# spcl/gms

Measured on AMD Instinct MI355X. Metric: edges-intersected/sec + achieved HBM GB/s, RMAT-26 triangle count @1/2/4/8 GPU, higher is better.
Workload: dtype int32 ids / uint64 counts

## Files before the change

### gms_amd/csrc/hip/device_graph.hip

```cpp
#include "device_graph.hpp"

#include <algorithm>
#include <mutex>
#include <array>
#include <chrono>
#include <cstdio>
#include <cstdlib>
#include <cstring>
#include <memory>
#include <new>
#include <random>

#include <rocprim/device/device_radix_sort.hpp>
#include <rocprim/device/device_scan.hpp>
#include <rocprim/device/device_segmented_radix_sort.hpp>
#include <rocprim/iterator/transform_iterator.hpp>

#include "../host/gmsx_internal.hpp"
#include "../host/tc_core_plan.hpp"
#include "kc4_mfma.hpp"

namespace gmsx {

Ctx &ctx() {
// ... 576 lines not shown
    uint32_t *c = cnt + p * kClasses;
    uint32_t run = 0;
    for (int k = 0; k < hub_end; ++k) { const uint32_t x = c[k]; c[k] = run; run += x; }
    hcnt[p] = run;
    run = 0;
    for (int k = hub_end; k < kClasses; ++k) { const uint32_t x = c[k]; c[k] = run; run += x; }
    tcnt[p] = run;
}

__global__ void k_ledge_count(int64_t first, int64_t end, const int32_t *__restrict__ order, const int64_t *__restrict__ toff, const int32_t *__restrict__ tadj,
                              const int32_t *__restrict__ tsplit, const int32_t *__restrict__ dplus, int32_t core, int64_t *__restrict__ cnt) {
    const int64_t pos = first + int64_t(blockIdx.x) * blockDim.x + threadIdx.x;
    if (pos > end) return;
    int64_t c = 0;
    if (pos < end) {
        const int32_t u = order[pos];
        const int64_t tb = toff[u];
        const int tl = int(toff[u + 1] - tb);
        if (u >= core)
            for (int i = tsplit[u]; i < tl; ++i) c += dplus[tadj[tb + i]] < kHeavy ? 1 : 0;
    }
    cnt[pos - first] = c;
}
__global__ void k_ledge_fill(int64_t first, int64_t end, const int32_t *__restrict__ order, const int64_t *__restrict__ hoff, const int64_t *__restrict__ toff,
                             const int32_t *__restrict__ tadj, const int32_t *__restrict__ tsplit, const int32_t *__restrict__ dplus,
                             int32_t core, const int64_t *__restrict__ ebeg, int nparts, int part, uint4 *__restrict__ ledge) {
    const int64_t pos = first + int64_t(blockIdx.x) * blockDim.x + threadIdx.x;
    if (pos >= end) return;
    const int32_t u = order[pos];
    if (u < core) return;
    const int64_t hb = hoff[u], tb = toff[u];
    const int tl = int(toff[u + 1] - tb);
    const unsigned long long hu = (unsigned long long)hb | ((unsigned long long)(hoff[u + 1] - hb) << 40);
    int64_t e = ebeg[pos - first];
    for (int i = tsplit[u]; i < tl; ++i) {
        const int32_t v = tadj[tb + i];
        if (dplus[v] >= kHeavy) continue;
        if (nparts <= 1 || shard_of(e, nparts) == part) {
            const unsigned long long tu = (unsigned long long)tb | ((unsigned long long)i << 40);
            const unsigned long long hv = (unsigned long long)hoff[v] | ((unsigned long long)(hoff[v + 1] - hoff[v]) << 40);
            const unsigned long long tv = (unsigned long long)toff[v] | ((unsigned long long)(toff[v + 1] - toff[v]) << 40);
            const int64_t slot = nparts <= 1 ? e : e / nparts;
            ledge[2 * slot] = make_uint4(uint32_t(hu), uint32_t(hu >> 32), uint32_t(tu), uint32_t(tu >> 32));
            ledge[2 * slot + 1] = make_uint4(uint32_t(hv), uint32_t(hv >> 32), uint32_t(tv), uint32_t(tv >> 32));
        }
        ++e;
    }
}

__device__ __forceinline__ uint32_t cut_hub_units(const uint32_t *__restrict__ spool, unsigned long long d, int below, int32_t v) {
    const uint32_t units = uint32_t(d) & 0x3fffffu, form = (uint32_t(d) >> 22) & 3u;
    if (form == kFormList) return min(units, uint32_t(below + 7) / 8u);
    if (form == kFormBitset) return min(units, uint32_t(v + 127) / 128u);
    const uint4 *row = reinterpret_cast<const uint4 *>(spool) + (d >> 24);
    uint32_t lo = 0, hi = units;
    while (lo < hi) {
        const uint32_t mid = (lo + hi) >> 1;
        if (int32_t(row[mid].x & 0xffffu) < v) lo = mid + 1; else hi = mid;
    }
    return lo;
}
__device__ __forceinline__ uint32_t cut_tail_units(const uint32_t *__restrict__ tpool, unsigned long long d, int below, int32_t v) {
    const uint32_t units = uint32_t(d) & 0x3fffffu, form = (uint32_t(d) >> 22) & 3u;
    if (form != kFormDelta) return min(units, uint32_t(below + 3) / 4u);
    const uint4 *row = reinterpret_cast<const uint4 *>(tpool) + (d >> 24);
    uint32_t lo = 0, hi = units;
    while (lo < hi) {
// ... 162 lines not shown
        *p = nullptr;
        return GMSX_ERR_DEVICE_MEM;
    }
    if (hipMalloc(reinterpret_cast<void **>(p), bytes) != hipSuccess) {
        (void)hipGetLastError();
        *p = nullptr;
        return GMSX_ERR_DEVICE_MEM;
    }
    if (g) g->device_bytes += int64_t(bytes);
    return GMSX_OK;
}

struct DevGuard {
    void *p;
    ~DevGuard() { (void)hipFree(p); }
};

static void free_tc(gmsx_graph *g) {
    auto drop = [](auto *&p) {
        (void)hipFree(p);
        p = nullptr;
    };
    drop(g->tsplit); drop(g->srow); drop(g->srow2); drop(g->ksplit); drop(g->spool); drop(g->trow); drop(g->htask.lo); drop(g->htask.hi); drop(g->ttask.lo); drop(g->ttask.hi); drop(g->hitem); drop(g->titem); drop(g->tunits);
    drop(g->ledge); drop(g->tpool); drop(g->shard_hitem); drop(g->shard_titem); drop(g->core_bits);
    g->tc_core = 0;
    g->shard_idx_part = g->shard_idx_nparts = -1;
    g->device_bytes -= g->tc_bytes;
    g->tc_bytes = 0;
    g->tc_ready = false;
    g->htask_entries = g->ttask_entries = g->hitems = g->titems = g->inline_hentries = g->inline_tentries = 0;
    g->n_ledge = g->ledge_total = 0;
    g->task_reverse = g->inline_units = g->spool_units = g->tpool_units = 0;
    g->stats_part = g->stats_nparts = -1;
}

static void free_graph(gmsx_graph *g) {
    if (!g) return;
    (void)hipFree(g->off);
    (void)hipFree(g->adj);
    (void)hipFree(g->newid);
    (void)hipFree(g->oldid);
    (void)hipFree(g->hoff);
    (void)hipFree(g->hadj);
    (void)hipFree(g->toff);
    (void)hipFree(g->tadj);
    (void)hipFree(g->bmoff);
    (void)hipFree(g->bmpool);
    (void)hipFree(g->tsplit);
    (void)hipFree(g->srow);
    (void)hipFree(g->srow2);
    (void)hipFree(g->ksplit);
    (void)hipFree(g->spool);
    (void)hipFree(g->trow);
    (void)hipFree(g->htask.lo);
    (void)hipFree(g->htask.hi);
    (void)hipFree(g->ttask.lo);
    (void)hipFree(g->ttask.hi);
    (void)hipFree(g->hitem);
    (void)hipFree(g->titem);
    (void)hipFree(g->tunits);
    (void)hipFree(g->shard_hitem);
    (void)hipFree(g->shard_titem);
    (void)hipFree(g->ledge);
    (void)hipFree(g->core_bits);
    (void)hipFree(g->tpool);
    (void)hipFree(g->dplus);
    (void)hipFree(g->order);
    (void)hipFree(g->kc_rel);
    (void)hipFree(g->kc_aoff);
    (void)hipFree(g->kc_arena);
    (void)hipFree(g->kc_rec);
    (void)hipFree(g->kc_item);
    (void)hipFree(g->kc_relt);
    (void)hipFree(g->kc_rect);
    (void)hipFree(g->kc_itemt);
    (void)hipFree(g->scratch);
    (void)hipFree(g->acc);
    delete g;
}

int exclusive_scan_i64(const int64_t *in, int64_t *out, int64_t count, hipStream_t s) {
    size_t tmp_bytes = 0;
    GMSX_HIP(rocprim::exclusive_scan(nullptr, tmp_bytes, in, out, int64_t(0), size_t(count), rocprim::plus<int64_t>(), s));
    void *tmp = nullptr;
    GMSX_HIP(hipMalloc(&tmp, tmp_bytes ? tmp_bytes : 8));
    DevGuard g_tmp{tmp};
// ... 502 lines not shown
        GMSX_HIP(hipMemcpy(&small_units, soff + n, sizeof(int64_t), hipMemcpyDeviceToHost));
        inline_t_base = big_units + small_units;
        g->tpool_units = inline_t_base + inline_t_units;
        if (g->tpool_units >= (int64_t(1) << 40)) return GMSX_ERR_DEVICE_MEM;
        if (int rc = dmalloc(&g->trow, n, g)) return rc;
        if (int rc = dmalloc(&g->tpool, (g->tpool_units + kPoolSlack) * 4, g)) return rc;
        GMSX_HIP(hipMemsetD32Async(reinterpret_cast<hipDeviceptr_t>(g->tpool), int(0xFFFFFFFEu), size_t(g->tpool_units + kPoolSlack) * 4, s));
        if (n > 0)
            hipLaunchKernelGGL(k_trow_fill, dim3(unsigned((n + 255) / 256)), dim3(256), 0, s, n, g->toff, g->tadj, uoff, soff, real, form, g->trow, g->tpool);
        GMSX_HIP(hipStreamSynchronize(s));
    }

    pt.mark("tail stream rows");
    if (n_work > 0) {
        GMSX_HIP(hipMemsetAsync(inl_h, 0, size_t(n + 1) * sizeof(unsigned long long), s));
        GMSX_HIP(hipMemsetAsync(inl_t, 0, size_t(n + 1) * sizeof(unsigned long long), s));
        hipLaunchKernelGGL(k_inline_rows<true>, dim3(grid_for_waves(n_work)), dim3(256), 0, s, int64_t(0), n_work, g->order, g->hoff, g->hadj, g->toff,
                           g->tadj, g->dplus, g->inline_limit, g->inline_first, g->tc_core, opos, g->shard_nparts, g->shard_part, inl_h, inl_t, ihoff, itoff, inline_h_base, reinterpret_cast<uint16_t *>(g->spool),
                           inline_t_base, reinterpret_cast<int32_t *>(g->tpool));
    }
    pt.mark("inline rows fill");
    {
        const int64_t nl = n_work - n_heavy;
        g->n_ledge = g->ledge_total = 0;
        if (nl > 0) {
            int64_t *ecnt = nullptr, *ebeg = nullptr;
            if (int rc = dmalloc(&ecnt, nl + 1, nullptr)) return rc;
            DevGuard g_ec{ecnt};
            if (int rc = dmalloc(&ebeg, nl + 1, nullptr)) return rc;
            DevGuard g_eb{ebeg};
            hipLaunchKernelGGL(k_ledge_count, dim3(unsigned(nl / 256 + 1)), dim3(256), 0, s, n_heavy, n_work, g->order, g->toff, g->tadj, g->tsplit, g->dplus, g->tc_core, ecnt);
            if (int rc = exclusive_scan_i64(ecnt, ebeg, nl + 1, s)) return rc;
            GMSX_HIP(hipMemcpy(&g->ledge_total, ebeg + nl, sizeof(int64_t), hipMemcpyDeviceToHost));
            const int np = g->shard_nparts > 1 ? g->shard_nparts : 1, pp = g->shard_nparts > 1 ? g->shard_part : 0;
            {
                const int64_t full = g->ledge_total / np, rem = g->ledge_total % np;
                g->n_ledge = np <= 1 ? g->ledge_total : full + (((full & 1) ? np - 1 - pp : pp) < rem ? 1 : 0);
            }
            if (int rc = dmalloc(&g->ledge, 2 * g->n_ledge + 2, g)) return rc;
            hipLaunchKernelGGL(k_ledge_fill, dim3(unsigned(nl / 256 + 1)), dim3(256), 0, s, n_heavy, n_work, g->order, g->hoff, g->toff, g->tadj, g->tsplit, g->dplus, g->tc_core, ebeg,
                               np, pp, g->ledge);
            GMSX_HIP(hipStreamSynchronize(s));
        }
    }
    pt.mark("light pivot list");
    {
        int two_sided = 1;
        if (const char *e = opt("TC_TWO_SIDED")) two_sided = std::atoi(e) != 0;
        const unsigned vb = unsigned(n / 256 + 1);
        const int64_t L = g->inline_limit;
        int64_t *lflag = nullptr, *lidx = nullptr;
        if (int rc = dmalloc(&lflag, L + 1, nullptr)) return rc;
        DevGuard g_lf{lflag};
        if (int rc = dmalloc(&lidx, L + 1, nullptr)) return rc;
        DevGuard g_li{lidx};
        hipLaunchKernelGGL(k_light_flags, dim3(unsigned(L / 256 + 1)), dim3(256), 0, s, L, g->dplus, lflag);
        if (int rc = exclusive_scan_i64(lflag, lidx, L + 1, s)) return rc;
        int64_t n_light_recv = 0;
        GMSX_HIP(hipMemcpy(&n_light_recv, lidx + L, sizeof(int64_t), hipMemcpyDeviceToHost));
        const int64_t n_recv = n_heavy + n_light_recv;
        int32_t *recv_v = nullptr;
        if (int rc = dmalloc(&recv_v, n_recv + 1, nullptr)) return rc;
        DevGuard g_rv{recv_v};
        if (std::max<int64_t>(n_heavy, L) > 0)
// ... 388 lines not shown
```

### gms_amd/csrc/hip/device_graph.hpp

```cpp
#pragma once
#include <hip/hip_runtime.h>

#include <cstdint>

#include "gmsx.h"
#include "gmsx_internal.hpp"

#if !defined(GMSX_DEV_HOOKS) &&                                                                                                               \
    (defined(GMSX_KC_NO_PROBE) || defined(GMSX_KC_NO_HITS) || defined(GMSX_KC_NO_TAIL) || defined(GMSX_KC_NO_INNER) || defined(GMSX_KC_CELLS_ONLY) ||   \
     defined(GMSX_KC_NO_ROWS) || defined(GMSX_KC_BUILD_ONLY) || defined(GMSX_KC_NO_SLAB_CALL) || defined(GMSX_KC_NO_PAIRS) || defined(GMSX_KC_SLAB_ROW_SCAN) || \
     defined(GMSX_BK_AB) || defined(GMSX_BK_NO_HIT_ATOMICS) || defined(GMSX_BK_STATS) || defined(GMSX_TC_NO_PROBE) || defined(GMSX_TC_STAGING_ONLY))
#error "A/B switches need -DGMSX_DEV_HOOKS (tools/ab_lib.sh sets it); the default build of libgmsx.so carries none of them"
#endif

struct __attribute__((aligned(64))) gmsx_tc_item {
    uint64_t bc;
    uint64_t cont;
    int32_t pivot;
    int32_t pos;
    uint32_t kind;
    uint16_t fbeg[4];
    uint32_t reserved[7];
};
static_assert(sizeof(gmsx_tc_item) == 64, "work item record = one 64-byte line");
constexpr uint32_t kTaskHubUnitsMax = (1u << 14) - 1, kTaskTailUnitsMax = (1u << 15) - 1;
struct TaskList {
    uint32_t *lo = nullptr;
    uint16_t *hi = nullptr;
    bool tail = false;
// ... 20 lines not shown
    uint16_t *hadj = nullptr;
    int64_t *toff = nullptr;
    int32_t *tadj = nullptr;
    int64_t *bmoff = nullptr;
    uint32_t *bmpool = nullptr;
    int32_t dense_limit = 0;
    int32_t bitset_limit = 0;
    unsigned long long *srow = nullptr;
    unsigned long long *srow2 = nullptr;
    int32_t *ksplit = nullptr;
    uint32_t *spool = nullptr;
    int64_t spool_units = 0;
    TaskList htask{nullptr, nullptr, false};
    TaskList ttask{nullptr, nullptr, true};
    int64_t htask_entries = 0, ttask_entries = 0;
    struct gmsx_tc_item *hitem = nullptr, *titem = nullptr;
    int64_t hitems = 0, titems = 0;
    int64_t inline_hentries = 0, inline_tentries = 0;
    mutable struct gmsx_tc_item *shard_hitem = nullptr, *shard_titem = nullptr;
    mutable int64_t shard_hitems = 0, shard_titems = 0;
    mutable int shard_idx_part = -1, shard_idx_nparts = -1;
    int32_t *tunits = nullptr;
    int64_t task_reverse = 0;
    uint4 *ledge = nullptr;
    int64_t n_ledge = 0, ledge_total = 0;
    uint32_t *core_bits = nullptr;
    int32_t tc_core = 0;
    mutable int core_bytes_k = -1, core_bytes_part = -1, core_bytes_nparts = -1;
    mutable uint64_t core_bytes = 0;
    int tc_hot_windows = 0;
    uint32_t tc_window_units = 1;
    int tc_hot_min = 0;
    int inline_first = 64;
    int32_t inline_limit = 0;
    int64_t inline_units = 0;
    unsigned long long *trow = nullptr;
    uint32_t *tpool = nullptr;
    int64_t tpool_units = 0;
    int32_t *tsplit = nullptr;
    int64_t dense_rows = 0, bmpool_words = 0;
    bool rows_sorted = false;
    int32_t *dplus = nullptr;
    int32_t *order = nullptr;
    int64_t hub_entries = 0, tail_entries = 0;
    int32_t max_dplus = 0;
    int32_t max_deg = 0;
    mutable bool kc_rev_tried = false;
    mutable uint32_t *kc_rel = nullptr;
// ... 89 lines not shown
    hipStream_t side[2] = {nullptr, nullptr};
    hipEvent_t ev_fork = nullptr, ev_join[2] = {nullptr, nullptr};
    int compute_units = 0;
};
Ctx &ctx();
int ensure_init();
int kclique_vertex_counts(const gmsx_graph *g, unsigned long long *d_counts, gmsx_stats *st);
int count_dplus_ge(const gmsx_graph *g, int32_t threshold, int64_t *out);
int exclusive_scan_i64(const int64_t *in, int64_t *out, int64_t count, hipStream_t s);
int ensure_tc(const gmsx_graph *g);
int ensure_tc_shard(const gmsx_graph *g, int part, int nparts);
int tc_shard_items(const gmsx_graph *g, int part, int nparts);
int tc_vertex_counts_device(const gmsx_graph *g, unsigned long long *d_counts, gmsx_stats *st);
int tc_full_partial(const gmsx_graph *g, int part, int nparts, uint64_t *partial, gmsx_stats *st);

__device__ __forceinline__ int uni32(int x) { return __builtin_amdgcn_readfirstlane(x); }
__device__ __forceinline__ uint32_t uni32(uint32_t x) { return uint32_t(__builtin_amdgcn_readfirstlane(int(x))); }
__device__ __forceinline__ int64_t uni64(int64_t x) {
    const uint32_t lo = uint32_t(__builtin_amdgcn_readfirstlane(int(uint32_t(uint64_t(x)))));
    const uint32_t hi = uint32_t(__builtin_amdgcn_readfirstlane(int(uint32_t(uint64_t(x) >> 32))));
    return int64_t((uint64_t(hi) << 32) | lo);
}
__device__ __forceinline__ unsigned long long uni64(unsigned long long x) { return (unsigned long long)uni64(int64_t(x)); }

#define GMSX_HIP(call)                                                    \
    do {                                                                  \
        hipError_t e_ = (call);                                           \
        if (e_ != hipSuccess) {                                           \
            (void)hipGetLastError();                                      \
            return e_ == hipErrorOutOfMemory ? GMSX_ERR_DEVICE_MEM : GMSX_ERR_KERNEL; \
        }                                                                 \
    } while (0)

}
```

### gms_amd/csrc/hip/tc.hip

```cpp
#include "device_graph.hpp"
#include "kc4_mfma.hpp"
#include "../host/tc_core_plan.hpp"

#include <algorithm>
#include <type_traits>
#include <rocprim/device/device_radix_sort.hpp>
#include <rocprim/device/device_reduce.hpp>
#include <rocprim/device/device_reduce_by_key.hpp>
#include <cstdio>
#include <cstdlib>
#include <cstring>

namespace gmsx {

static constexpr int kAccSlots = 64;
static constexpr int kAccStride = 16;

struct __attribute__((packed, aligned(4))) u4u { uint32_t x, y, z, w; };

__device__ __forceinline__ int64_t readlane64(int64_t x, int l) {
    const uint32_t lo = __builtin_amdgcn_readlane(uint32_t(uint64_t(x)), l);
    const uint32_t hi = __builtin_amdgcn_readlane(uint32_t(uint64_t(x) >> 32), l);
    return int64_t((uint64_t(hi) << 32) | lo);
}
// ... 511 lines not shown
__global__ __launch_bounds__(256) __attribute__((amdgpu_waves_per_eu(TAIL ? GMSX_TC_TAIL_MIN_WAVES : GMSX_TC_HUB_MIN_WAVES, 8))) void k_tc_items(
    const uint16_t *__restrict__ hadj, const int32_t *__restrict__ tadj, const uint32_t *__restrict__ pool, const TaskList task,
    const gmsx_tc_item *__restrict__ items, int n_items, unsigned int *__restrict__ qhead, unsigned long long *__restrict__ acc) {
    __shared__ __attribute__((aligned(16))) ItemLds L;
    const int tid = threadIdx.x;
    unsigned long long total = 0;
    item_loop<TAIL>(L, hadj, tadj, pool, task, items, n_items, qhead, total);
    block_add(total, L.red, tid & 63, tid >> 6, tid, acc);
}

template <int K>
__device__ __forceinline__ uint32_t ror_in_row(uint32_t x) {
    if constexpr (K == 0) return x;
    else return uint32_t(__builtin_amdgcn_mov_dpp(int(x), 0x120 + K, 0xf, 0xf, false));
}
__device__ __forceinline__ bool row_has(uint32_t a, uint32_t x) {
    bool m = false;
#define GMSX_ROT(K) m |= a == ror_in_row<K>(x);
    GMSX_ROT(0) GMSX_ROT(1) GMSX_ROT(2) GMSX_ROT(3) GMSX_ROT(4) GMSX_ROT(5) GMSX_ROT(6) GMSX_ROT(7)
    GMSX_ROT(8) GMSX_ROT(9) GMSX_ROT(10) GMSX_ROT(11) GMSX_ROT(12) GMSX_ROT(13) GMSX_ROT(14) GMSX_ROT(15)
#undef GMSX_ROT
    return m;
}
struct LightRows {
    uint32_t ah[4], at[4], bh[4], bt[4];
};
struct LightRec {
    uint4 r0, r1;
};
__global__ __launch_bounds__(256) void k_tc_light(const uint16_t *__restrict__ hadj, const int32_t *__restrict__ tadj, const uint4 *__restrict__ ledge, int nparts,
                                                  int part, int64_t count, unsigned long long *__restrict__ acc) {
    __shared__ unsigned long long red[4];
    const int tid = threadIdx.x, lane = tid & 63, wave = tid >> 6, sub = lane & 15;
    const int64_t ngroups = int64_t(gridDim.x) * 16, g0 = int64_t(blockIdx.x) * 16 + (tid >> 4);
    const int64_t trips = (count + ngroups - 1) / ngroups;
    auto load_rec = [&](int64_t t) -> LightRec {
        const int64_t k = g0 + t * ngroups;
        const int64_t kk = k < count ? k : 0;
        const int64_t e = nparts <= 1 ? kk : kk * nparts + ((kk & 1) ? nparts - 1 - part : part);
        LightRec r;
        r.r0 = ledge[2 * e];
        r.r1 = ledge[2 * e + 1];
        if (k >= count) {
            r.r0.y &= 0xffu;
            r.r0.w &= 0xffu;
            r.r1.y &= 0xffu;
            r.r1.w &= 0xffu;
        }
        return r;
    };
    auto wave_max = [](int x) {
        return max(max(__builtin_amdgcn_readlane(x, 0), __builtin_amdgcn_readlane(x, 16)), max(__builtin_amdgcn_readlane(x, 32), __builtin_amdgcn_readlane(x, 48)));
    };
    auto load_rows = [&](const LightRec &r) -> LightRows {
        const int64_t hu = int64_t((uint64_t(r.r0.y & 0xffu) << 32) | r.r0.x), tu = int64_t((uint64_t(r.r0.w & 0xffu) << 32) | r.r0.z);
        const int64_t hv = int64_t((uint64_t(r.r1.y & 0xffu) << 32) | r.r1.x), tv = int64_t((uint64_t(r.r1.w & 0xffu) << 32) | r.r1.z);
        const int hlu = int(r.r0.y >> 8), tlu = int(r.r0.w >> 8), hlv = int(r.r1.y >> 8), tlv = int(r.r1.w >> 8);
        const int more = wave_max((max(max(hlu, hlv), max(tlu, tlv)) + 15) >> 4);
        LightRows w;
        w.ah[0] = hadj[hlu ? hu + min(sub, hlu - 1) : 0];
        w.bh[0] = hadj[hlv ? hv + min(sub, hlv - 1) : 0];
        w.at[0] = uint32_t(tadj[tlu ? tu + min(sub, tlu - 1) : 0]);
        w.bt[0] = uint32_t(tadj[tlv ? tv + min(sub, tlv - 1) : 0]);
#pragma unroll
        for (int k = 1; k < 4; ++k) {
            w.ah[k] = w.bh[k] = w.at[k] = w.bt[k] = 0;
            if (k < more) {
                const int i = sub + 16 * k;
                w.ah[k] = hadj[hlu ? hu + min(i, hlu - 1) : 0];
                w.bh[k] = hadj[hlv ? hv + min(i, hlv - 1) : 0];
                w.at[k] = uint32_t(tadj[tlu ? tu + min(i, tlu - 1) : 0]);
                w.bt[k] = uint32_t(tadj[tlv ? tv + min(i, tlv - 1) : 0]);
            }
        }
        return w;
    };
    unsigned long long total = 0;
    if (trips > 0) {
        LightRec rec = load_rec(0);
        LightRows rows = load_rows(rec);
        LightRec rec_n = load_rec(1);
        for (int64_t t = 0; t < trips; ++t) {
            const LightRows rows_n = load_rows(rec_n);
            const LightRec rec_nn = load_rec(t + 2);
            const int hlu = int(rec.r0.y >> 8), tlu = int(rec.r0.w >> 8), hlv = int(rec.r1.y >> 8), tlv = int(rec.r1.w >> 8);
            const int nah = wave_max((hlu + 15) >> 4), nbh = wave_max((hlv + 15) >> 4), nat = wave_max((tlu + 15) >> 4), nbt = wave_max((tlv + 15) >> 4);
            uint32_t c = 0;
#pragma unroll
            for (int ka = 0; ka < 4; ++ka) {
                if (ka >= nah) break;
                const int ia = sub + 16 * ka;
                const uint32_t a = (ia < hlu && rows.ah[ka] != 0xFFFFu) ? rows.ah[ka] : 0xFFFFFFFFu;
                bool m = false;
#pragma unroll
                for (int kb = 0; kb < 4; ++kb) {
                    if (kb >= nbh) break;
                    const int ib = sub + 16 * kb;
                    const uint32_t x = (ib < hlv && rows.bh[kb] != 0xFFFFu) ? rows.bh[kb] : 0xFFFFFFFEu;
                    m |= row_has(a, x);
                }
                c += m ? 1u : 0u;
            }
#pragma unroll
            for (int ka = 0; ka < 4; ++ka) {
                if (ka >= nat) break;
                const int ia = sub + 16 * ka;
                const uint32_t a = ia < tlu ? rows.at[ka] : 0xFFFFFFFFu;
                bool m = false;
#pragma unroll
                for (int kb = 0; kb < 4; ++kb) {
                    if (kb >= nbt) break;
                    const int ib = sub + 16 * kb;
                    const uint32_t x = ib < tlv ? rows.bt[kb] : 0xFFFFFFFEu;
                    m |= row_has(a, x);
                }
                c += m ? 1u : 0u;
            }
            total += c;
            rec = rec_n;
            rows = rows_n;
            rec_n = rec_nn;
        }
    }
    block_add(total, red, lane, wave, tid, acc);
}

__global__ __launch_bounds__(1024) void k_tc_core(const uint32_t *__restrict__ bits, int WS, int K, int nb, int nblk, int part, int nparts,
                                                  unsigned long long *__restrict__ acc) {
    __shared__ unsigned long long red[16];
    auto lane_id = [] { return int(__builtin_amdgcn_mbcnt_hi(~0u, __builtin_amdgcn_mbcnt_lo(~0u, 0u))); };
    const int wave = uni32(int(threadIdx.x) >> 6);
    const int x = blockIdx.x & 7, y = blockIdx.x >> 3, Y = int(gridDim.x) >> 3;
    const int Q = 16 * Y, q = y * 16 + wave;
    const int ns = (nblk - part + nparts - 1) / nparts;
    uint32_t cnt = 0;
    for (int j = 0;; ++j) {
        const int sidx = (8 * j + ((j & 1) ? 7 - x : x)) * Q + q;
        if (sidx >= ns) break;
        const int t = sidx * nparts + part;
        int c = int((__builtin_sqrtf(8.0f * float(t) + 1.0f) - 1.0f) * 0.5f);
        while (c * (c + 1) / 2 > t) --c;
        while ((c + 1) * (c + 2) / 2 <= t) ++c;
        const int bj = nb - 1 - c, bi = bj + (t - c * (c + 1) / 2);
        int lane = lane_id();
// ... 20 lines not shown
    const int lane = threadIdx.x & 63;
    const int64_t wave0 = (int64_t(blockIdx.x) * blockDim.x + threadIdx.x) >> 6;
    const int64_t nwaves = (int64_t(gridDim.x) * blockDim.x) >> 6;
    unsigned long long units = 0, probes = 0, bytes = 0;
    for (int64_t pos = wave0; pos < end; pos += nwaves) {
        if (nparts > 1 && shard_of(pos, nparts) != part) continue;
        const int32_t u = order[pos];
        const int du = dplus[u];
        if (du >= kHeavy) {
            if (lane == 0) units += (unsigned long long)tunits[pos];
            if (u < core) {
                if (lane == 0) units += (unsigned long long)du;
                continue;
            }
            const int hl = min(int(hoff[u + 1] - hoff[u]), inline_first), tl = min(int(toff[u + 1] - toff[u]), inline_first - hl);
            int32_t v = -1;
            if (lane < hl) {
                const uint32_t x = hadj[hoff[u] + lane];
                if (x != 0xFFFFu) v = int32_t(x);
            } else if (lane - hl < tl) v = tadj[toff[u] + lane - hl];
            if (v >= 0 && lane > 0 && (v < inline_limit || dplus[v] >= kHeavy)) ++units;
            continue;
        }
        const int hl = int(hoff[u + 1] - hoff[u]);
        if (lane == 0) units += (unsigned long long)du;
        if (du < 2 || u < core) continue;
        for (int64_t j = toff[u] + lane; j < toff[u + 1]; j += 64) {
            const int32_t v = tadj[j];
            if (v < inline_limit || dplus[v] >= kHeavy) continue;
            const unsigned long long hv = (unsigned long long)(hoff[v + 1] - hoff[v]), tv = (unsigned long long)(toff[v + 1] - toff[v]);
            bytes += 32ull + 2ull * hl + 4ull * (unsigned long long)(j - toff[u]) + 2ull * hv + 4ull * tv;
            probes += hv + tv;
        }
    }
    for (int s = 32; s > 0; s >>= 1) {
        units += __shfl_down(units, s);
        probes += __shfl_down(probes, s);
        bytes += __shfl_down(bytes, s);
    }
    if (lane == 0) {
        if (units) atomicAdd(&out[0], units);
        if (probes) atomicAdd(&out[1], probes);
        if (bytes) atomicAdd(&out[2], bytes);
    }
}
__global__ __launch_bounds__(256) void k_tc_item_stats(const int64_t *__restrict__ coff, int bytes_per_id, int tail, const TaskList task,
                                                       const gmsx_tc_item *__restrict__ items, int64_t n_items, int nparts, int part,
                                                       unsigned long long *__restrict__ out) {
    const int lane = threadIdx.x & 63;
    const int64_t wave0 = (int64_t(blockIdx.x) * blockDim.x + threadIdx.x) >> 6;
    const int64_t nwaves = (int64_t(gridDim.x) * blockDim.x) >> 6;
    unsigned long long probes = 0, bytes = 0;
    auto slots = [tail](unsigned long long d) -> unsigned long long {
        const unsigned long long n = d & 0x3fffffull, f = (d >> 22) & 3ull;
// ... 1 lines not shown
    };
    for (int64_t q = wave0; q < n_items; q += nwaves) {
        const gmsx_tc_item &it = items[q];
        if (nparts > 1 && shard_of(it.pos, nparts) != part) continue;
        const int ne = int(it.bc >> 40);
        const int64_t b = int64_t(it.bc & 0xffffffffffull);
        if (lane == 0) bytes += (unsigned long long)bytes_per_id * (unsigned long long)(coff[it.pivot + 1] - coff[it.pivot]);
        for (int i = lane; i < ne; i += 64) {
            const unsigned long long d = task.get(b + i);
            bytes += 6ull + 16ull * (d & 0x3fffffull);
            probes += slots(d);
        }
    }
    for (int s = 32; s > 0; s >>= 1) {
        probes += __shfl_down(probes, s);
        bytes += __shfl_down(bytes, s);
    }
    if (lane == 0) {
        if (probes) atomicAdd(&out[1], probes);
        if (bytes) atomicAdd(&out[2], bytes);
    }
}

__global__ __launch_bounds__(256) void k_tc_breakdown(const int64_t *__restrict__ hoff, const int64_t *__restrict__ toff, const int32_t *__restrict__ tadj,
                                                      const int32_t *__restrict__ dplus, const int32_t *__restrict__ order,
                                                      const TaskList htask, const gmsx_tc_item *__restrict__ hitem, int64_t hitems,
                                                      const TaskList ttask, const gmsx_tc_item *__restrict__ titem, int64_t titems,
                                                      int32_t inline_limit, int32_t core, int64_t first_light, int64_t end_light,
                                                      unsigned long long *__restrict__ out) {
    const int lane = threadIdx.x & 63;
    const int64_t wave0 = (int64_t(blockIdx.x) * blockDim.x + threadIdx.x) >> 6;
    const int64_t nwaves = (int64_t(gridDim.x) * blockDim.x) >> 6;
    unsigned long long c[15] = {0, 0, 0, 0, 0, 0, 0, 0, 0, 0, 0, 0, 0, 0, 0};
    for (int64_t q = wave0; q < hitems + titems; q += nwaves) {
        const bool tail = q >= hitems;
        const gmsx_tc_item &it = tail ? titem[q - hitems] : hitem[q];
        const TaskList task = tail ? ttask : htask;
        const int ne = int(it.bc >> 40);
        const int64_t b0 = int64_t(it.bc & 0xffffffffffull);
        if (lane == 0) {
            c[6] += tail ? 4ull * (unsigned long long)(toff[it.pivot + 1] - toff[it.pivot]) : 2ull * (unsigned long long)(hoff[it.pivot + 1] - hoff[it.pivot]);
            c[11] += (unsigned long long)ne;
            c[13] += 1;
        }
        for (int i = lane; i < ne; i += 64) {
            const unsigned long long d = task.get(b0 + i);
            const unsigned long long db = 16ull * (d & 0x3fffffull);
            const int fd = int((d >> 22) & 3);
            if (tail) c[fd == kFormDelta ? 4 : 3] += db;
            else c[fd == kFormList ? 0 : fd == kFormBitset ? 1 : 2] += db;
            c[5] += 6;
        }
    }
    for (int64_t pos = first_light + wave0; pos < end_light; pos += nwaves) {
        const int32_t u = order[pos];
        if (u < core) continue;
        const int64_t tb0 = toff[u], te = toff[u + 1];
        const unsigned long long hl = (unsigned long long)(hoff[u + 1] - hoff[u]);
        for (int64_t j = tb0 + lane; j < te; j += 64) {
            const int32_t v = tadj[j];
            if (v < inline_limit || dplus[v] >= kHeavy) continue;
            c[8] += 2ull * (unsigned long long)(hoff[v + 1] - hoff[v]);
            c[9] += 4ull * (unsigned long long)(toff[v + 1] - toff[v]);
            c[10] += 32ull + 2ull * hl + 4ull * (unsigned long long)(j - tb0);
            c[14] += 1;
        }
    }
    for (int k = 0; k < 15; ++k) {
        unsigned long long x = c[k];
        for (int s = 32; s > 0; s >>= 1) x += __shfl_down(x, s);
        if (lane == 0 && x) atomicAdd(&out[k], x);
    }
}

__device__ __forceinline__ int hist_bin(unsigned long long units) {
    if (units <= 16) return int(units) - 1;
    int b = 16;
    for (unsigned long long lim = 32; units > lim && b < 23; lim <<= 1) ++b;
    return b;
}
__global__ __launch_bounds__(256) void k_tc_comember_keys(const TaskList htask, const gmsx_tc_item *__restrict__ hitem, int64_t hitems, int batch,
                                                         unsigned long long *__restrict__ keys, uint32_t *__restrict__ vals, unsigned long long *__restrict__ sums) {
    unsigned long long ents = 0, units = 0;
    for (int64_t i = blockIdx.x; i < hitems; i += gridDim.x) {
        const gmsx_tc_item it = hitem[i];
        const unsigned long long first = it.bc & 0xffffffffffull;
        const int n = int(it.bc >> 40);
// ... 234 lines not shown
        auto grid = [&](int64_t n, int wgs) {
            return unsigned(std::max<int64_t>(1, std::min<int64_t>((n + kGrab - 1) / kGrab, int64_t(cus) * (wgs_env > 0 ? wgs_env : wgs))));
        };
        if (n_hitems > 0) {
            hipLaunchKernelGGL(k_tc_items<false>, dim3(grid(n_hitems, GMSX_TC_HUB_MIN_WAVES)), dim3(256), 0, s, g->hadj, g->tadj, g->spool, g->htask, hitem, int(n_hitems), qhead, acc);
            ++launches;
        }
        if (n_titems > 0) {
            hipLaunchKernelGGL(k_tc_items<true>, dim3(grid(n_titems, GMSX_TC_TAIL_MIN_WAVES)), dim3(256), 0, s, g->hadj, g->tadj, g->tpool, g->ttask, titem, int(n_titems),
                               qhead + kQueueStride, acc);
            ++launches;
        }
    } else {
        if (n_hitems > 0) {
            hipLaunchKernelGGL(k_tc_block, dim3(unsigned(n_hitems)), dim3(256), 0, s, g->hoff, g->hadj, g->spool, g->htask, hitem, acc);
            ++launches;
        }
        if (n_titems > 0) {
            hipLaunchKernelGGL(k_tc_tail, dim3(unsigned(n_titems)), dim3(256), 0, side_tail ? c.side[0] : s, g->toff, g->tadj, g->tpool, g->ttask, titem, acc);
            ++launches;
        }
    }
    if (cnt_light > 0) {
        const int64_t blocks = std::min<int64_t>((cnt_light + 15) / 16, int64_t(cus) * 8);
        hipLaunchKernelGGL(k_tc_light, dim3(unsigned(blocks)), dim3(256), 0, side_light ? c.side[1] : s, g->hadj, g->tadj, g->ledge, strided ? nparts : 1,
                           strided ? part : 0, cnt_light, acc);
        ++launches;
    }
    for (int i = 0; i < 2; ++i)
        if (join.armed[i]) {
            join.armed[i] = false;
            GMSX_HIP(hipEventRecord(c.ev_join[i], c.side[i]));
            GMSX_HIP(hipStreamWaitEvent(s, c.ev_join[i], 0));
        }
    GMSX_HIP(hipEventRecord(c.ev[2], s));
    GMSX_HIP(hipGetLastError());

    const bool need_stats = st && !(g->stats_part == part && g->stats_nparts == nparts);
    if (need_stats) {
        if (g->n > 0) {
            const int64_t blocks = std::min<int64_t>((g->n + 3) / 4, cap_blocks);
            hipLaunchKernelGGL(k_tc_stats, dim3(unsigned(blocks)), dim3(256), 0, s, g->hoff, g->hadj, g->toff, g->tadj, g->dplus, g->order,
                               g->tunits, g->inline_limit, g->inline_first, g->tc_core, g->n, nparts, part, acc + kAccSlots * kAccStride);
        }
        if (g->hitems > 0)
            hipLaunchKernelGGL(k_tc_item_stats, dim3(unsigned(std::min<int64_t>((g->hitems + 3) / 4, cap_blocks))), dim3(256), 0, s, g->hoff, 2, 0, g->htask, g->hitem,
                               g->hitems, nparts, part, acc + kAccSlots * kAccStride);
        if (g->titems > 0)
// ... 33 lines not shown

using namespace gmsx;

extern "C" {

int gmsx_tc_divisor(int algo) { return algo == GMSX_TC_FULL ? 3 : 1; }

int gmsx_tc_stream_breakdown(const gmsx_graph *g, uint64_t *out21) {
    return gmsx::guard([&]() -> int {
        if (!g || !out21) return GMSX_ERR_INVALID;
        if (int rc = ensure_init()) return rc;
        if (int rc = ensure_tc(g)) return rc;
        hipStream_t s = ctx().stream;
        std::memset(out21, 0, 21 * sizeof(uint64_t));
        if (g->n == 0) return GMSX_OK;
        int64_t n_block = 0, n_work = 0;
        if (int rc = count_dplus_ge(g, kHeavy, &n_block)) return rc;
        if (int rc = count_dplus_ge(g, 2, &n_work)) return rc;
        unsigned long long *acc = nullptr;
        GMSX_HIP(hipMalloc(reinterpret_cast<void **>(&acc), 21 * 8));
        struct Guard { void *p; ~Guard() { (void)hipFree(p); } } g1{acc};
        GMSX_HIP(hipMemsetAsync(acc, 0, 21 * 8, s));
        const int cus = ctx().compute_units > 0 ? ctx().compute_units : 256;
        hipLaunchKernelGGL(k_tc_breakdown, dim3(unsigned(cus * 16)), dim3(256), 0, s, g->hoff, g->toff, g->tadj, g->dplus, g->order, g->htask,
                           g->hitem, g->hitems, g->ttask, g->titem, g->titems, g->inline_limit, g->tc_core, n_block, n_work, acc);
        GMSX_HIP(hipMemcpyAsync(out21, acc, 21 * 8, hipMemcpyDeviceToHost, s));
        GMSX_HIP(hipStreamSynchronize(s));
        GMSX_HIP(hipGetLastError());
        out21[7] = uint64_t(g->inline_units) * 16ull;
        out21[12] = uint64_t(g->inline_hentries + g->inline_tentries);
        out21[15] = core_bytes_of(g, 0, 1);
        out21[16] = uint64_t(g->tc_core);
        return GMSX_OK;
    });
}

int gmsx_tc_row_histogram(const gmsx_graph *g, uint64_t *out256) {
    return gmsx::guard([&]() -> int {
        uint64_t *out248 = out256;
        if (!g || !out248) return GMSX_ERR_INVALID;
        if (int rc = ensure_init()) return rc;
        if (int rc = ensure_tc(g)) return rc;
        hipStream_t s = ctx().stream;
        std::memset(out248, 0, 256 * sizeof(uint64_t));
        if (g->n == 0) return GMSX_OK;
        unsigned long long *acc = nullptr;
        GMSX_HIP(hipMalloc(reinterpret_cast<void **>(&acc), 256 * 8));
// ... 91 lines not shown
```

Baseline: 16.11 billion.

## Pack light-edge rows into contiguous pooled records with compact descriptors

Preprocessing now copies each light edge's four neighbor row slices (hub u, tail prefix u, hub v, tail v) into one contiguous packed record in a new pool, indexed by an 8-byte descriptor. Before, a 32-byte record pointed into the scattered hadj/tadj arrays. The light kernel now reads one descriptor plus one contiguous record instead of gathering from four scattered rows. This targets random-access gather cost and over-fetch. It also strips hub sentinels at build time, double-buffers the loop, and sizes the grid by queried occupancy. In exchange it duplicates adjacency data, which costs more memory and preprocessing time, and caps row lengths at 8 bits.

```diff
diff --git a/gms_amd/csrc/hip/device_graph.hip b/gms_amd/csrc/hip/device_graph.hip
--- a/gms_amd/csrc/hip/device_graph.hip
+++ b/gms_amd/csrc/hip/device_graph.hip
@@ -622,27 +622,55 @@
     }
     cnt[pos - first] = c;
 }
-__global__ void k_ledge_fill(int64_t first, int64_t end, const int32_t *__restrict__ order, const int64_t *__restrict__ hoff, const int64_t *__restrict__ toff,
-                             const int32_t *__restrict__ tadj, const int32_t *__restrict__ tsplit, const int32_t *__restrict__ dplus,
-                             int32_t core, const int64_t *__restrict__ ebeg, int nparts, int part, uint4 *__restrict__ ledge) {
+__global__ void k_ledge_units(int64_t first, int64_t end, const int32_t *__restrict__ order, const int64_t *__restrict__ hoff, const uint16_t *__restrict__ hadj,
+                              const int64_t *__restrict__ toff, const int32_t *__restrict__ tadj, const int32_t *__restrict__ tsplit, const int32_t *__restrict__ dplus,
+                              int32_t core, const int64_t *__restrict__ ebeg, int nparts, int part, int64_t *__restrict__ cnt) {
     const int64_t pos = first + int64_t(blockIdx.x) * blockDim.x + threadIdx.x;
+    if (pos > end) return;
+    int64_t c = 0;
+    if (pos < end) {
+        const int32_t u = order[pos];
+        if (u >= core) {
+            const int64_t tb = toff[u];
+            const int tl = int(toff[u + 1] - tb), hu = hub_ids(hoff, hadj, u);
+            int64_t e = ebeg[pos - first];
+            for (int i = tsplit[u]; i < tl; ++i) {
+                const int32_t v = tadj[tb + i];
+                if (dplus[v] >= kHeavy) continue;
+                if (nparts <= 1 || shard_of(e, nparts) == part) c += light_units(light_pack_lens(hu, i, hub_ids(hoff, hadj, v), int(toff[v + 1] - toff[v])));
+                ++e;
+            }
+        }
+    }
+    cnt[pos - first] = c;
+}
+__global__ __launch_bounds__(256) void k_ledge_fill(int64_t first, int64_t end, const int32_t *__restrict__ order, const int64_t *__restrict__ hoff,
+                                                    const uint16_t *__restrict__ hadj, const int64_t *__restrict__ toff, const int32_t *__restrict__ tadj,
+                                                    const int32_t *__restrict__ tsplit, const int32_t *__restrict__ dplus, int32_t core,
+                                                    const int64_t *__restrict__ ebeg, const int64_t *__restrict__ ubeg, int nparts, int part,
+                                                    uint2 *__restrict__ ldesc, uint4 *__restrict__ lpool) {
+    const int64_t pos = first + ((int64_t(blockIdx.x) * blockDim.x + threadIdx.x) >> 4);
+    const int sub = threadIdx.x & 15;
     if (pos >= end) return;
     const int32_t u = order[pos];
     if (u < core) return;
     const int64_t hb = hoff[u], tb = toff[u];
-    const int tl = int(toff[u + 1] - tb);
-    const unsigned long long hu = (unsigned long long)hb | ((unsigned long long)(hoff[u + 1] - hb) << 40);
-    int64_t e = ebeg[pos - first];
+    const int tl = int(toff[u + 1] - tb), hu = hub_ids(hoff, hadj, u);
+    int64_t e = ebeg[pos - first], unit = ubeg[pos - first];
     for (int i = tsplit[u]; i < tl; ++i) {
         const int32_t v = tadj[tb + i];
         if (dplus[v] >= kHeavy) continue;
         if (nparts <= 1 || shard_of(e, nparts) == part) {
-            const unsigned long long tu = (unsigned long long)tb | ((unsigned long long)i << 40);
-            const unsigned long long hv = (unsigned long long)hoff[v] | ((unsigned long long)(hoff[v + 1] - hoff[v]) << 40);
-            const unsigned long long tv = (unsigned long long)toff[v] | ((unsigned long long)(toff[v + 1] - toff[v]) << 40);
-            const int64_t slot = nparts <= 1 ? e : e / nparts;
-            ledge[2 * slot] = make_uint4(uint32_t(hu), uint32_t(hu >> 32), uint32_t(tu), uint32_t(tu >> 32));
-            ledge[2 * slot + 1] = make_uint4(uint32_t(hv), uint32_t(hv >> 32), uint32_t(tv), uint32_t(tv >> 32));
+            const int64_t hvb = hoff[v], tvb = toff[v];
+            const int hv = hub_ids(hoff, hadj, v), tv = int(toff[v + 1] - tvb);
+            const uint32_t lens = light_pack_lens(hu, i, hv, tv);
+            if (sub == 0) ldesc[nparts <= 1 ? e : e / nparts] = make_uint2(uint32_t(unit), lens);
+            uint4 *rec = lpool + unit;
+            for (int k = sub; k < hu; k += 16) light_put(rec, lens, 0, k, hadj[hb + k]);
+            for (int k = sub; k < i; k += 16) light_put(rec, lens, 1, k, uint32_t(tadj[tb + k]));
+            for (int k = sub; k < hv; k += 16) light_put(rec, lens, 2, k, hadj[hvb + k]);
+            for (int k = sub; k < tv; k += 16) light_put(rec, lens, 3, k, uint32_t(tadj[tvb + k]));
+            unit += light_units(lens);
         }
         ++e;
     }
@@ -851,14 +879,14 @@
         p = nullptr;
     };
     drop(g->tsplit); drop(g->srow); drop(g->srow2); drop(g->ksplit); drop(g->spool); drop(g->trow); drop(g->htask.lo); drop(g->htask.hi); drop(g->ttask.lo); drop(g->ttask.hi); drop(g->hitem); drop(g->titem); drop(g->tunits);
-    drop(g->ledge); drop(g->tpool); drop(g->shard_hitem); drop(g->shard_titem); drop(g->core_bits);
+    drop(g->ldesc); drop(g->lpool); drop(g->tpool); drop(g->shard_hitem); drop(g->shard_titem); drop(g->core_bits);
     g->tc_core = 0;
     g->shard_idx_part = g->shard_idx_nparts = -1;
     g->device_bytes -= g->tc_bytes;
     g->tc_bytes = 0;
     g->tc_ready = false;
     g->htask_entries = g->ttask_entries = g->hitems = g->titems = g->inline_hentries = g->inline_tentries = 0;
-    g->n_ledge = g->ledge_total = 0;
+    g->n_ledge = g->ledge_total = g->lpool_units = 0;
     g->task_reverse = g->inline_units = g->spool_units = g->tpool_units = 0;
     g->stats_part = g->stats_nparts = -1;
 }
@@ -890,7 +918,8 @@
     (void)hipFree(g->tunits);
     (void)hipFree(g->shard_hitem);
     (void)hipFree(g->shard_titem);
-    (void)hipFree(g->ledge);
+    (void)hipFree(g->ldesc);
+    (void)hipFree(g->lpool);
     (void)hipFree(g->core_bits);
     (void)hipFree(g->tpool);
     (void)hipFree(g->dplus);
@@ -1439,13 +1468,15 @@
     pt.mark("inline rows fill");
     {
         const int64_t nl = n_work - n_heavy;
-        g->n_ledge = g->ledge_total = 0;
+        g->n_ledge = g->ledge_total = g->lpool_units = 0;
         if (nl > 0) {
-            int64_t *ecnt = nullptr, *ebeg = nullptr;
+            int64_t *ecnt = nullptr, *ebeg = nullptr, *ubeg = nullptr;
             if (int rc = dmalloc(&ecnt, nl + 1, nullptr)) return rc;
             DevGuard g_ec{ecnt};
             if (int rc = dmalloc(&ebeg, nl + 1, nullptr)) return rc;
             DevGuard g_eb{ebeg};
+            if (int rc = dmalloc(&ubeg, nl + 1, nullptr)) return rc;
+            DevGuard g_ub{ubeg};
             hipLaunchKernelGGL(k_ledge_count, dim3(unsigned(nl / 256 + 1)), dim3(256), 0, s, n_heavy, n_work, g->order, g->toff, g->tadj, g->tsplit, g->dplus, g->tc_core, ecnt);
             if (int rc = exclusive_scan_i64(ecnt, ebeg, nl + 1, s)) return rc;
             GMSX_HIP(hipMemcpy(&g->ledge_total, ebeg + nl, sizeof(int64_t), hipMemcpyDeviceToHost));
@@ -1454,9 +1485,17 @@
                 const int64_t full = g->ledge_total / np, rem = g->ledge_total % np;
                 g->n_ledge = np <= 1 ? g->ledge_total : full + (((full & 1) ? np - 1 - pp : pp) < rem ? 1 : 0);
             }
-            if (int rc = dmalloc(&g->ledge, 2 * g->n_ledge + 2, g)) return rc;
-            hipLaunchKernelGGL(k_ledge_fill, dim3(unsigned(nl / 256 + 1)), dim3(256), 0, s, n_heavy, n_work, g->order, g->hoff, g->toff, g->tadj, g->tsplit, g->dplus, g->tc_core, ebeg,
-                               np, pp, g->ledge);
+            hipLaunchKernelGGL(k_ledge_units, dim3(unsigned(nl / 256 + 1)), dim3(256), 0, s, n_heavy, n_work, g->order, g->hoff, g->hadj, g->toff, g->tadj, g->tsplit, g->dplus,
+                               g->tc_core, ebeg, np, pp, ecnt);
+            if (int rc = exclusive_scan_i64(ecnt, ubeg, nl + 1, s)) return rc;
+            GMSX_HIP(hipMemcpy(&g->lpool_units, ubeg + nl, sizeof(int64_t), hipMemcpyDeviceToHost));
+            if (g->lpool_units + kPoolSlack >= (int64_t(1) << 32)) return GMSX_ERR_DEVICE_MEM;
+            if (int rc = dmalloc(&g->ldesc, g->n_ledge + 2, g)) return rc;
+            if (int rc = dmalloc(&g->lpool, g->lpool_units + kPoolSlack, g)) return rc;
+            GMSX_HIP(hipMemsetAsync(g->ldesc, 0, size_t(g->n_ledge + 2) * sizeof(uint2), s));
+            GMSX_HIP(hipMemsetAsync(g->lpool, kLightFillByte, size_t(g->lpool_units + kPoolSlack) * sizeof(uint4), s));
+            hipLaunchKernelGGL(k_ledge_fill, dim3(unsigned(nl / 16 + 1)), dim3(256), 0, s, n_heavy, n_work, g->order, g->hoff, g->hadj, g->toff, g->tadj, g->tsplit, g->dplus,
+                               g->tc_core, ebeg, ubeg, np, pp, g->ldesc, g->lpool);
             GMSX_HIP(hipStreamSynchronize(s));
         }
     }
diff --git a/gms_amd/csrc/hip/device_graph.hpp b/gms_amd/csrc/hip/device_graph.hpp
--- a/gms_amd/csrc/hip/device_graph.hpp
+++ b/gms_amd/csrc/hip/device_graph.hpp
@@ -5,6 +5,7 @@
 
 #include "gmsx.h"
 #include "gmsx_internal.hpp"
+#include "light_record.hpp"
 
 #if !defined(GMSX_DEV_HOOKS) &&                                                                                                               \
     (defined(GMSX_KC_NO_PROBE) || defined(GMSX_KC_NO_HITS) || defined(GMSX_KC_NO_TAIL) || defined(GMSX_KC_NO_INNER) || defined(GMSX_KC_CELLS_ONLY) ||   \
@@ -71,8 +72,9 @@
     mutable int shard_idx_part = -1, shard_idx_nparts = -1;
     int32_t *tunits = nullptr;
     int64_t task_reverse = 0;
-    uint4 *ledge = nullptr;
-    int64_t n_ledge = 0, ledge_total = 0;
+    uint2 *ldesc = nullptr;
+    uint4 *lpool = nullptr;
+    int64_t n_ledge = 0, ledge_total = 0, lpool_units = 0;
     uint32_t *core_bits = nullptr;
     int32_t tc_core = 0;
     mutable int core_bytes_k = -1, core_bytes_part = -1, core_bytes_nparts = -1;
@@ -208,6 +210,11 @@
     return int64_t((uint64_t(hi) << 32) | lo);
 }
 __device__ __forceinline__ unsigned long long uni64(unsigned long long x) { return (unsigned long long)uni64(int64_t(x)); }
+__device__ __forceinline__ int hub_ids(const int64_t *__restrict__ hoff, const uint16_t *__restrict__ hadj, int32_t v) {
+    const int64_t b = hoff[v];
+    const int hl = int(hoff[v + 1] - b);
+    return hl > 0 && hadj[b + hl - 1] == 0xFFFFu ? hl - 1 : hl;
+}
 
 #define GMSX_HIP(call)                                                    \
     do {                                                                  \
diff --git a/gms_amd/csrc/hip/light_record.hpp b/gms_amd/csrc/hip/light_record.hpp
--- /dev/null
+++ b/gms_amd/csrc/hip/light_record.hpp
@@ -0,0 +1,40 @@
+#pragma once
+#include <cstdint>
+
+#if defined(__HIPCC__)
+#define GMSX_HD __host__ __device__
+#else
+#define GMSX_HD
+#endif
+
+namespace gmsx {
+
+static constexpr int kLightParts = 4;
+static constexpr int kLightMaxLen = 63;
+static constexpr uint8_t kLightFillByte = 0xFF;
+
+GMSX_HD inline uint32_t light_pack_lens(int hu, int tu, int hv, int tv) {
+    return uint32_t(hu) | (uint32_t(tu) << 8) | (uint32_t(hv) << 16) | (uint32_t(tv) << 24);
+}
+GMSX_HD inline int light_len(uint32_t lens, int part) { return int((lens >> (8 * part)) & 0xffu); }
+GMSX_HD inline bool light_part_is_hub(int part) { return (part & 1) == 0; }
+GMSX_HD inline int light_part_dword(uint32_t lens, int part) {
+    const int hu = light_len(lens, 0), tu = light_len(lens, 1), hv = light_len(lens, 2);
+    const int o1 = (hu + 1) >> 1, o2 = o1 + tu, o3 = o2 + ((hv + 1) >> 1);
+    return part == 0 ? 0 : part == 1 ? o1 : part == 2 ? o2 : o3;
+}
+GMSX_HD inline int light_dwords(uint32_t lens) { return light_part_dword(lens, 3) + light_len(lens, 3); }
+GMSX_HD inline int light_units(uint32_t lens) { return (light_dwords(lens) + 3) >> 2; }
+GMSX_HD inline int light_id_byte(uint32_t lens, int part, int i) {
+    return 4 * light_part_dword(lens, part) + (light_part_is_hub(part) ? 2 : 4) * i;
+}
+GMSX_HD inline int light_hub_bytes(uint32_t lens) { return 2 * (light_len(lens, 0) + light_len(lens, 2)); }
+GMSX_HD inline int light_tail_bytes(uint32_t lens) { return 4 * (light_len(lens, 1) + light_len(lens, 3)); }
+GMSX_HD inline int light_fill_bytes(uint32_t lens) { return 16 * light_units(lens) - light_hub_bytes(lens) - light_tail_bytes(lens); }
+GMSX_HD inline void light_put(void *rec, uint32_t lens, int part, int i, uint32_t id) {
+    unsigned char *p = static_cast<unsigned char *>(rec) + light_id_byte(lens, part, i);
+    if (light_part_is_hub(part)) *reinterpret_cast<uint16_t *>(p) = uint16_t(id);
+    else *reinterpret_cast<uint32_t *>(p) = id;
+}
+
+}
diff --git a/gms_amd/csrc/hip/tc.hip b/gms_amd/csrc/hip/tc.hip
--- a/gms_amd/csrc/hip/tc.hip
+++ b/gms_amd/csrc/hip/tc.hip
@@ -557,104 +557,101 @@
 #undef GMSX_ROT
     return m;
 }
-struct LightRows {
+struct LightSet {
     uint32_t ah[4], at[4], bh[4], bt[4];
+    uint32_t lens;
+    int n[4];
 };
-struct LightRec {
-    uint4 r0, r1;
-};
-__global__ __launch_bounds__(256) void k_tc_light(const uint16_t *__restrict__ hadj, const int32_t *__restrict__ tadj, const uint4 *__restrict__ ledge, int nparts,
-                                                  int part, int64_t count, unsigned long long *__restrict__ acc) {
+__global__ __launch_bounds__(256) void k_tc_light(const uint2 *__restrict__ ldesc, const uint4 *__restrict__ lpool, int nparts, int part, int64_t count,
+                                                  unsigned long long *__restrict__ acc) {
     __shared__ unsigned long long red[4];
     const int tid = threadIdx.x, lane = tid & 63, wave = tid >> 6, sub = lane & 15;
     const int64_t ngroups = int64_t(gridDim.x) * 16, g0 = int64_t(blockIdx.x) * 16 + (tid >> 4);
     const int64_t trips = (count + ngroups - 1) / ngroups;
-    auto load_rec = [&](int64_t t) -> LightRec {
+    auto load_desc = [&](int64_t t) -> uint2 {
         const int64_t k = g0 + t * ngroups;
         const int64_t kk = k < count ? k : 0;
         const int64_t e = nparts <= 1 ? kk : kk * nparts + ((kk & 1) ? nparts - 1 - part : part);
-        LightRec r;
-        r.r0 = ledge[2 * e];
-        r.r1 = ledge[2 * e + 1];
-        if (k >= count) {
-            r.r0.y &= 0xffu;
-            r.r0.w &= 0xffu;
-            r.r1.y &= 0xffu;
-            r.r1.w &= 0xffu;
-        }
-        return r;
+        uint2 d = ldesc[e];
+        if (k >= count) d.y = 0;
+        return d;
     };
-    auto wave_max = [](int x) {
-        return max(max(__builtin_amdgcn_readlane(x, 0), __builtin_amdgcn_readlane(x, 16)), max(__builtin_amdgcn_readlane(x, 32), __builtin_amdgcn_readlane(x, 48)));
-    };
-    auto load_rows = [&](const LightRec &r) -> LightRows {
-        const int64_t hu = int64_t((uint64_t(r.r0.y & 0xffu) << 32) | r.r0.x), tu = int64_t((uint64_t(r.r0.w & 0xffu) << 32) | r.r0.z);
-        const int64_t hv = int64_t((uint64_t(r.r1.y & 0xffu) << 32) | r.r1.x), tv = int64_t((uint64_t(r.r1.w & 0xffu) << 32) | r.r1.z);
-        const int hlu = int(r.r0.y >> 8), tlu = int(r.r0.w >> 8), hlv = int(r.r1.y >> 8), tlv = int(r.r1.w >> 8);
-        const int more = wave_max((max(max(hlu, hlv), max(tlu, tlv)) + 15) >> 4);
-        LightRows w;
-        w.ah[0] = hadj[hlu ? hu + min(sub, hlu - 1) : 0];
-        w.bh[0] = hadj[hlv ? hv + min(sub, hlv - 1) : 0];
-        w.at[0] = uint32_t(tadj[tlu ? tu + min(sub, tlu - 1) : 0]);
-        w.bt[0] = uint32_t(tadj[tlv ? tv + min(sub, tlv - 1) : 0]);
+    auto load_set = [&](const uint2 d, LightSet &w) {
+        const uint32_t lens = d.y;
+        const uint32_t y0 = uint32_t(__builtin_amdgcn_readlane(int(lens), 0)), y1 = uint32_t(__builtin_amdgcn_readlane(int(lens), 16));
+        const uint32_t y2 = uint32_t(__builtin_amdgcn_readlane(int(lens), 32)), y3 = uint32_t(__builtin_amdgcn_readlane(int(lens), 48));
+        w.lens = lens;
+        auto smax = [](int a, int b) {
+            int m = max(a, b);
+            asm volatile("" : "+s"(m));
+            return m;
+        };
+#pragma unroll
+        for (int p = 0; p < kLightParts; ++p) w.n[p] = (smax(smax(light_len(y0, p), light_len(y1, p)), smax(light_len(y2, p), light_len(y3, p))) + 15) >> 4;
+        const int more = smax(smax(w.n[0], w.n[1]), smax(w.n[2], w.n[3]));
+        const unsigned char *rec = reinterpret_cast<const unsigned char *>(lpool + d.x);
+        const int cah = max(light_len(lens, 0) - 1, 0), cat = max(light_len(lens, 1) - 1, 0), cbh = max(light_len(lens, 2) - 1, 0), cbt = max(light_len(lens, 3) - 1, 0);
+        auto hub = [&](int p, int i) { return uint32_t(*reinterpret_cast<const uint16_t *>(rec + light_id_byte(lens, p, i))); };
+        auto tail = [&](int p, int i) { return *reinterpret_cast<const uint32_t *>(rec + light_id_byte(lens, p, i)); };
+        w.ah[0] = hub(0, min(sub, cah));
+        w.at[0] = tail(1, min(sub, cat));
+        w.bh[0] = hub(2, min(sub, cbh));
+        w.bt[0] = tail(3, min(sub, cbt));
 #pragma unroll
         for (int k = 1; k < 4; ++k) {
             w.ah[k] = w.bh[k] = w.at[k] = w.bt[k] = 0;
             if (k < more) {
                 const int i = sub + 16 * k;
-                w.ah[k] = hadj[hlu ? hu + min(i, hlu - 1) : 0];
-                w.bh[k] = hadj[hlv ? hv + min(i, hlv - 1) : 0];
-                w.at[k] = uint32_t(tadj[tlu ? tu + min(i, tlu - 1) : 0]);
-                w.bt[k] = uint32_t(tadj[tlv ? tv + min(i, tlv - 1) : 0]);
+                w.ah[k] = hub(0, min(i, cah));
+                w.at[k] = tail(1, min(i, cat));
+                w.bh[k] = hub(2, min(i, cbh));
+                w.bt[k] = tail(3, min(i, cbt));
             }
         }
-        return w;
+    };
+    auto compare = [&](const LightSet &w) -> uint32_t {
+        const int hlu = light_len(w.lens, 0), tlu = light_len(w.lens, 1), hlv = light_len(w.lens, 2), tlv = light_len(w.lens, 3);
+        uint32_t c = 0;
+#pragma unroll
+        for (int ka = 0; ka < 4; ++ka) {
+            if (ka >= w.n[0]) break;
+            const uint32_t a = sub + 16 * ka < hlu ? w.ah[ka] : 0xFFFFFFFFu;
+            bool m = false;
+#pragma unroll
+            for (int kb = 0; kb < 4; ++kb) {
+                if (kb >= w.n[2]) break;
+                const uint32_t x = sub + 16 * kb < hlv ? w.bh[kb] : 0xFFFFFFFEu;
+                m |= row_has(a, x);
+            }
+            c += m ? 1u : 0u;
+        }
+#pragma unroll
+        for (int ka = 0; ka < 4; ++ka) {
+            if (ka >= w.n[1]) break;
+            const uint32_t a = sub + 16 * ka < tlu ? w.at[ka] : 0xFFFFFFFFu;
+            bool m = false;
+#pragma unroll
+            for (int kb = 0; kb < 4; ++kb) {
+                if (kb >= w.n[3]) break;
+                const uint32_t x = sub + 16 * kb < tlv ? w.bt[kb] : 0xFFFFFFFEu;
+                m |= row_has(a, x);
+            }
+            c += m ? 1u : 0u;
+        }
+        return c;
     };
     unsigned long long total = 0;
     if (trips > 0) {
-        LightRec rec = load_rec(0);
-        LightRows rows = load_rows(rec);
-        LightRec rec_n = load_rec(1);
-        for (int64_t t = 0; t < trips; ++t) {
-            const LightRows rows_n = load_rows(rec_n);
-            const LightRec rec_nn = load_rec(t + 2);
-            const int hlu = int(rec.r0.y >> 8), tlu = int(rec.r0.w >> 8), hlv = int(rec.r1.y >> 8), tlv = int(rec.r1.w >> 8);
-            const int nah = wave_max((hlu + 15) >> 4), nbh = wave_max((hlv + 15) >> 4), nat = wave_max((tlu + 15) >> 4), nbt = wave_max((tlv + 15) >> 4);
-            uint32_t c = 0;
-#pragma unroll
-            for (int ka = 0; ka < 4; ++ka) {
-                if (ka >= nah) break;
-                const int ia = sub + 16 * ka;
-                const uint32_t a = (ia < hlu && rows.ah[ka] != 0xFFFFu) ? rows.ah[ka] : 0xFFFFFFFFu;
-                bool m = false;
-#pragma unroll
-                for (int kb = 0; kb < 4; ++kb) {
-                    if (kb >= nbh) break;
-                    const int ib = sub + 16 * kb;
-                    const uint32_t x = (ib < hlv && rows.bh[kb] != 0xFFFFu) ? rows.bh[kb] : 0xFFFFFFFEu;
-                    m |= row_has(a, x);
-                }
-                c += m ? 1u : 0u;
-            }
-#pragma unroll
-            for (int ka = 0; ka < 4; ++ka) {
-                if (ka >= nat) break;
-                const int ia = sub + 16 * ka;
-                const uint32_t a = ia < tlu ? rows.at[ka] : 0xFFFFFFFFu;
-                bool m = false;
-#pragma unroll
-                for (int kb = 0; kb < 4; ++kb) {
-                    if (kb >= nbt) break;
-                    const int ib = sub + 16 * kb;
-                    const uint32_t x = ib < tlv ? rows.bt[kb] : 0xFFFFFFFEu;
-                    m |= row_has(a, x);
-                }
-                c += m ? 1u : 0u;
-            }
-            total += c;
-            rec = rec_n;
-            rows = rows_n;
-            rec_n = rec_nn;
+        LightSet A, B;
+        load_set(load_desc(0), A);
+        uint2 dn = load_desc(1);
+        for (int64_t t = 0; t < trips; t += 2) {
+            load_set(dn, B);
+            dn = load_desc(t + 2);
+            total += compare(A);
+            load_set(dn, A);
+            dn = load_desc(t + 3);
+            total += compare(B);
         }
     }
     block_add(total, red, lane, wave, tid, acc);
@@ -721,14 +718,14 @@
             if (v >= 0 && lane > 0 && (v < inline_limit || dplus[v] >= kHeavy)) ++units;
             continue;
         }
-        const int hl = int(hoff[u + 1] - hoff[u]);
         if (lane == 0) units += (unsigned long long)du;
         if (du < 2 || u < core) continue;
+        const int hu = hub_ids(hoff, hadj, u);
         for (int64_t j = toff[u] + lane; j < toff[u + 1]; j += 64) {
             const int32_t v = tadj[j];
             if (v < inline_limit || dplus[v] >= kHeavy) continue;
             const unsigned long long hv = (unsigned long long)(hoff[v + 1] - hoff[v]), tv = (unsigned long long)(toff[v + 1] - toff[v]);
-            bytes += 32ull + 2ull * hl + 4ull * (unsigned long long)(j - toff[u]) + 2ull * hv + 4ull * tv;
+            bytes += 8ull + 16ull * (unsigned long long)light_units(light_pack_lens(hu, int(j - toff[u]), hub_ids(hoff, hadj, v), int(tv)));
             probes += hv + tv;
         }
     }
@@ -776,7 +773,7 @@
     }
 }
 
-__global__ __launch_bounds__(256) void k_tc_breakdown(const int64_t *__restrict__ hoff, const int64_t *__restrict__ toff, const int32_t *__restrict__ tadj,
+__global__ __launch_bounds__(256) void k_tc_breakdown(const int64_t *__restrict__ hoff, const uint16_t *__restrict__ hadj, const int64_t *__restrict__ toff, const int32_t *__restrict__ tadj,
                                                       const int32_t *__restrict__ dplus, const int32_t *__restrict__ order,
                                                       const TaskList htask, const gmsx_tc_item *__restrict__ hitem, int64_t hitems,
                                                       const TaskList ttask, const gmsx_tc_item *__restrict__ titem, int64_t titems,
@@ -810,13 +807,14 @@
         const int32_t u = order[pos];
         if (u < core) continue;
         const int64_t tb0 = toff[u], te = toff[u + 1];
-        const unsigned long long hl = (unsigned long long)(hoff[u + 1] - hoff[u]);
+        const int hu = hub_ids(hoff, hadj, u);
         for (int64_t j = tb0 + lane; j < te; j += 64) {
             const int32_t v = tadj[j];
             if (v < inline_limit || dplus[v] >= kHeavy) continue;
-            c[8] += 2ull * (unsigned long long)(hoff[v + 1] - hoff[v]);
-            c[9] += 4ull * (unsigned long long)(toff[v + 1] - toff[v]);
-            c[10] += 32ull + 2ull * hl + 4ull * (unsigned long long)(j - tb0);
+            const uint32_t lens = light_pack_lens(hu, int(j - tb0), hub_ids(hoff, hadj, v), int(toff[v + 1] - toff[v]));
+            c[8] += (unsigned long long)light_hub_bytes(lens);
+            c[9] += (unsigned long long)light_tail_bytes(lens);
+            c[10] += 8ull + (unsigned long long)light_fill_bytes(lens);
             c[14] += 1;
         }
     }
@@ -1097,8 +1095,13 @@
         }
     }
     if (cnt_light > 0) {
-        const int64_t blocks = std::min<int64_t>((cnt_light + 15) / 16, int64_t(cus) * 8);
-        hipLaunchKernelGGL(k_tc_light, dim3(unsigned(blocks)), dim3(256), 0, side_light ? c.side[1] : s, g->hadj, g->tadj, g->ledge, strided ? nparts : 1,
+        static const int per_cu = [] {
+            int nb = 0;
+            if (hipOccupancyMaxActiveBlocksPerMultiprocessor(&nb, k_tc_light, 256, 0) != hipSuccess) (void)hipGetLastError();
+            return nb >= 1 && nb <= 8 ? nb : 8;
+        }();
+        const int64_t blocks = std::min<int64_t>((cnt_light + 15) / 16, int64_t(cus) * per_cu);
+        hipLaunchKernelGGL(k_tc_light, dim3(unsigned(blocks)), dim3(256), 0, side_light ? c.side[1] : s, g->ldesc, g->lpool, strided ? nparts : 1,
                            strided ? part : 0, cnt_light, acc);
         ++launches;
     }
@@ -1178,7 +1181,7 @@
         struct Guard { void *p; ~Guard() { (void)hipFree(p); } } g1{acc};
         GMSX_HIP(hipMemsetAsync(acc, 0, 21 * 8, s));
         const int cus = ctx().compute_units > 0 ? ctx().compute_units : 256;
-        hipLaunchKernelGGL(k_tc_breakdown, dim3(unsigned(cus * 16)), dim3(256), 0, s, g->hoff, g->toff, g->tadj, g->dplus, g->order, g->htask,
+        hipLaunchKernelGGL(k_tc_breakdown, dim3(unsigned(cus * 16)), dim3(256), 0, s, g->hoff, g->hadj, g->toff, g->tadj, g->dplus, g->order, g->htask,
                            g->hitem, g->hitems, g->ttask, g->titem, g->titems, g->inline_limit, g->tc_core, n_block, n_work, acc);
         GMSX_HIP(hipMemcpyAsync(out21, acc, 21 * 8, hipMemcpyDeviceToHost, s));
         GMSX_HIP(hipStreamSynchronize(s));
```

Result: no change. 16.22 billion, median of 6 (+0.7%).
